# sanderslab/magellanmapper

Measured on AMD Instinct MI355X. Metric: Mvoxels/s, 2048x2048x1024 uint16 stack, 5-sigma LoG blob detection, higher is better.
Workload: dtype f16x2 MFMA (f32 accumulate) + 16-bit fixed-point intermediates; f64 re-score of every candidate

## Files before the change

### magellanmapper_amd/csrc/mmx_api.hip

```cpp

#include <atomic>
#include <cstdio>
#include <cstdlib>
#include <cstring>

#include "mmx_common.h"

int mmx_launch_generic_pass(int pass, const mmx_volume* vol, const mmx_block* d_blocks, int n_blocks,
                            int max_vox, int64_t slot_elems, const float* w0, const float* w2, int radius,
                            const float* in1, const float* in2, float* out1, float* out2, hipStream_t s);
int mmx_launch_peaks(const float* d_log, int n_sigma, int64_t sigma_stride, const mmx_block* d_blocks,
                     int n_blocks, int max_vox, int64_t slot_elems, float thr, float eps,
                     mmx_cand* d_cands, uint32_t cap, uint32_t* d_count, hipStream_t stream);
int mmx_launch_peaks_sparse(const float* d_log, const unsigned long long* d_mask, int n_sigma,
                            int64_t sigma_stride, const mmx_block* d_blocks, int n_blocks, int max_vox,
                            int64_t slot_elems, float thr, float eps, mmx_cand* d_cands, uint32_t cap,
                            uint32_t* d_count, int quads, hipStream_t stream);

#include <mutex>
#include <vector>

namespace {
thread_local char g_hip_err[256] = "";

// ... 211 lines not shown
    int kind; hipStream_t s;
    pass_scope(int k, hipStream_t st) : kind(k), s(st) { if (k >= 0) mmx_time_begin(k, st); }
    ~pass_scope() { if (kind >= 0) mmx_time_end(kind, s); }
};

int fused_passes(const mmx_log_call& c, const mmx_route& r, const mmx_batch_geom& g, const pass_weights& w)
{
    const mmx_volume* vol = c.vol;
    const int radius = c.radius, n_blocks = c.n_blocks;
    const int64_t slot_elems = c.slot_elems;
    hipStream_t s = c.stream;
    float* t0 = c.d_work;
    float* t1 = c.d_work + (int64_t)n_blocks * slot_elems;
    mmx_taps_f32 tzz = taps(w.z0, w.z2, radius), txx = taps(w.y0, w.y2, radius), tyy = taps(w.x0, w.x2, radius);
    const bool tiled = r.family == MMX_ROUTE_TILED;
    const mmx_zx6_plan& plan = g.plan;
    int rc;
    if (r.makes_copy) {
        mmx_timed_scope ts(MMX_K_ZXPACK, s);
        rc = mmx_launch_zx6_pack(vol, c.d_blocks, c.h_blocks, n_blocks, plan, c.d_work, s);
        if (rc != MMX_OK) return launched(rc, "mmx_launch_zx6_pack", "voxel copy of the tiled path");
    }
    { mmx_timed_scope ts(MMX_K_ZX, s);
      if (tiled)
          rc = mmx_launch_zx6(vol, c.d_blocks, c.h_blocks, n_blocks, plan, txx, radius, c.d_work,
                              r.q16 ? (float)(1.0 / r.bp) : 0.f, r.q16 ? (float)(1.0 / r.bq) : 0.f, s);
      else
          rc = mmx_launch_zx2(vol, c.d_blocks, n_blocks, g.max_ny, g.max_px, slot_elems, tzz, txx, radius, t0, t1, s); }
    if (rc != MMX_OK) return launched(rc, tiled ? "mmx_launch_zx6" : "mmx_launch_zx2", "fused passes");
    { mmx_timed_scope ts(MMX_K_Y2, s);
      unsigned long long* d_mask = r.layout ? (unsigned long long*)c.d_nms_mask : nullptr;
      const float cp = r.q16 ? (float)(r.bp / 65535.0) : 0.f, cq = r.q16 ? (float)(r.bq / 32767.0) : 0.f;
      if (r.y_kernel == MMX_Y_YM)
          rc = mmx_launch_ym(c.d_blocks, n_blocks, plan, slot_elems, tyy, radius, c.d_work, cp, cq, c.d_log, d_mask,
                             c.nms_lo, c.nms_eps, s);
      else if (r.y_kernel == MMX_Y_Y6)
          rc = mmx_launch_y6(c.d_blocks, n_blocks, plan, slot_elems, tyy, radius, c.d_work,
                             reinterpret_cast<const float*>(reinterpret_cast<const char*>(c.d_work) + plan.q_off), cp, cq,
                             c.d_log, d_mask, c.nms_lo, c.nms_eps, s);
      else
          rc = mmx_launch_y2(c.d_blocks, n_blocks, g.max_ycols, slot_elems, tyy, radius, t0, t1, c.d_log, d_mask, c.nms_lo,
                             c.nms_eps, s); }
    return launched(rc, r.y_kernel == MMX_Y_YM ? "mmx_launch_ym" : (r.y_kernel == MMX_Y_Y6 ? "mmx_launch_y6" : "mmx_launch_y2"),
                    "fused passes");
}

int wide_passes(const mmx_log_call& c, const mmx_route& r, const pass_weights& w)
{
    const int radius = c.radius, n_blocks = c.n_blocks;
    const int64_t slot_elems = c.slot_elems;
    hipStream_t s = c.stream;
    float* t0 = c.d_work;
    float* t1 = t0 + (int64_t)n_blocks * slot_elems;
    float* t2 = t1 + (int64_t)n_blocks * slot_elems;
    float* t3 = t2 + (int64_t)n_blocks * slot_elems;
    unsigned long long* d_mask = r.layout ? (unsigned long long*)c.d_nms_mask : nullptr;
    int rc;
    { mmx_timed_scope ts(MMX_K_WIDE, s);
      rc = mmx_launch_wide_pass(0, c.vol, c.d_blocks, c.h_blocks, n_blocks, slot_elems, w.z0, w.z2, radius, nullptr, nullptr,
                                t2, t3, nullptr, 0.f, 0.f, s); }
    if (rc == MMX_OK) {
        mmx_timed_scope ts(MMX_K_WIDE, s);
        rc = mmx_launch_wide_pass(1, c.vol, c.d_blocks, c.h_blocks, n_blocks, slot_elems, w.y0, w.y2, radius, t2, t3, t0, t1,
                                  nullptr, 0.f, 0.f, s);
    }
    if (rc == MMX_OK) {
        mmx_timed_scope ts(MMX_K_WIDE, s);
// ... 196 lines not shown
```

### magellanmapper_amd/csrc/mmx_common.h

```cpp
#pragma once

#include <hip/hip_runtime.h>
#include <stdint.h>

#include "../../include/mmx.h"

#define MMX_WG 256
#define MMX_MAX_GRID_X 2147483647

struct mmx_taps_f32 {
    float w0[MMX_MAX_RADIUS_FAST + 1];
    float w2[MMX_MAX_RADIUS_FAST + 1];
};

__host__ __device__ __forceinline__ int mmx_reflect(int i, int n)
{
    if (n == 1) return 0;
    const int period = 2 * n;
    i %= period;
    if (i < 0) i += period;
    return i < n ? i : period - 1 - i;
}

int mmx_launch_zpass(const mmx_volume* vol, const mmx_block* d_blocks, int n_blocks, int max_cols,
                     int64_t slot_elems, const mmx_taps_f32& taps, int radius,
                     float* d_gz, float* d_gzz, hipStream_t stream);
int mmx_launch_ypass(const mmx_block* d_blocks, int n_blocks, int max_cols, int64_t slot_elems,
                     const mmx_taps_f32& taps, int radius, const float* d_gz, const float* d_gzz,
                     float* d_a, float* d_bc, hipStream_t stream);
int mmx_launch_xpass(const mmx_block* d_blocks, int n_blocks, int max_rows, int max_nx,
                     int64_t slot_elems, const mmx_taps_f32& taps, int radius,
                     const float* d_a, const float* d_bc, float* d_log, hipStream_t stream);

int mmx_launch_zx2(const mmx_volume* vol, const mmx_block* d_blocks, int n_blocks, int max_ny, int max_px,
                   int64_t slot_elems, const mmx_taps_f32& tz, const mmx_taps_f32& tx, int radius,
                   float* d_p, float* d_q, hipStream_t s);
struct mmx_zx6_plan {
    int64_t tile_stride;
    int64_t pack_stride;
    int64_t q_off, tab_off, pack_off;
    int64_t tab_bytes;
    int max_tiles;
    int max_rowtiles;
};
int mmx_zx6_plan_make(const mmx_block* h_blocks, int n_blocks, int64_t slot_elems, int voxel_dtype, mmx_zx6_plan* plan);
int mmx_launch_zx6_pack(const mmx_volume* vol, const mmx_block* d_blocks, const mmx_block* h_blocks, int n_blocks,
                        const mmx_zx6_plan& plan, void* d_work, hipStream_t stream);
int mmx_launch_zx6(const mmx_volume* vol, const mmx_block* d_blocks, const mmx_block* h_blocks, int n_blocks,
                   const mmx_zx6_plan& plan, const mmx_taps_f32& tx, int radius, void* d_work, float qp, float qq,
                   hipStream_t stream);
int mmx_launch_y6(const mmx_block* d_blocks, int n_blocks, const mmx_zx6_plan& plan, int64_t slot_elems,
                  const mmx_taps_f32& taps, int radius, const float* d_p, const float* d_q, float cp, float cq,
                  float* d_log, unsigned long long* d_mask, float nms_lo, float nms_eps, hipStream_t stream);
int mmx_launch_ym(const mmx_block* d_blocks, int n_blocks, const mmx_zx6_plan& plan, int64_t slot_elems,
                  const mmx_taps_f32& taps, int radius, const float* d_p, float cp, float cq,
                  float* d_log, unsigned long long* d_mask, float nms_lo, float nms_eps, hipStream_t stream);
int mmx_launch_y2(const mmx_block* d_blocks, int n_blocks, int max_cols, int64_t slot_elems,
                  const mmx_taps_f32& taps, int radius, const float* d_p, const float* d_q,
                  float* d_log, unsigned long long* d_mask, float nms_lo, float nms_eps, hipStream_t stream);

int mmx_launch_wide_pass(int pass, const mmx_volume* vol, const mmx_block* d_blocks, const mmx_block* h_blocks, int n_blocks,
                         int64_t slot_elems, const float* w0, const float* w2, int radius,
                         const float* in1, const float* in2, float* out1, float* out2,
                         unsigned long long* d_mask, float nms_lo, float nms_eps, hipStream_t s);

struct mmx_batch_geom {
    int status;
    bool bad_block;
    int min_nz, min_ny, min_nx, max_ny, max_nx, max_px;
    int max_zcols, max_ycols, max_rows, max_vox;
    int64_t max_lane_in;
    bool rows_fit, quads_fit;
    mmx_zx6_plan plan;
    int plan_status;
};
void mmx_batch_geom_make(const mmx_volume* vol, const mmx_block* h_blocks, int n_blocks, int64_t slot_elems, mmx_batch_geom* g);

#include "mmx_route.h"

struct mmx_log_call {
    const mmx_volume* vol; const mmx_block* d_blocks; const mmx_block* h_blocks; int n_blocks; int64_t slot_elems;
    const double* h_w0; const double* h_w2; int radius; double norm;
    float* d_log; float* d_work; uint64_t* d_nms_mask; float nms_lo, nms_eps; int* h_mask_written;
    int zx_mode; int* h_zx_path; hipStream_t stream;
};
int mmx_log_scale_check(const mmx_log_call& c);
int mmx_log_scale_run(const mmx_log_call& c, const mmx_batch_geom& g, const mmx_route& r);
int mmx_zx_pack_geom(const mmx_volume* vol, const mmx_block* d_blocks, const mmx_block* h_blocks, int n_blocks,
// ... 16 lines not shown
```

### magellanmapper_amd/csrc/mmx_fused4.hip

```cpp

#include <algorithm>
#include <type_traits>

#include "mmx_common.h"

typedef _Float16 h2_4 __attribute__((ext_vector_type(2)));
typedef _Float16 h8_4 __attribute__((ext_vector_type(8)));
typedef float f2_4 __attribute__((ext_vector_type(2)));
typedef float f4_4 __attribute__((ext_vector_type(4)));
typedef unsigned u4_4 __attribute__((ext_vector_type(4)));
typedef unsigned u2_4 __attribute__((ext_vector_type(2)));

#define MMX_ZX4_MAXCLS 8
#ifndef ZX4_ST_AUX
#define ZX4_ST_AUX 0
#endif
#ifndef ZX4_LD_AUX
#define ZX4_LD_AUX 0
#endif

struct mmx_zx4_cfg {
    float w0[MMX_MAX_RADIUS_FAST + 1];
    float w2[MMX_MAX_RADIUS_FAST + 1];
    float xscale;
// ... 28 lines not shown
template <int NKX, int LA> struct cls4 {
    static constexpr int R8 = NKX == 1 ? 8 : (LA == 1 ? 16 : 24);
    static __host__ __device__ constexpr int xstart(int c)
    {
        const int lo = 16 * c - R8;
        const int al = lo & ~31;
        return (al + 32 * NKX >= 16 * c + 16 + R8) ? al : lo;
    }
    static constexpr bool SPLIT = LA == 2;
    static constexpr int NKZ = 2;
    static constexpr int NT = 4;
};

__device__ __forceinline__ unsigned pack_h2(float a, float b)
{
    const f2_4 v = {a, b};
    return __builtin_bit_cast(unsigned, __builtin_convertvector(v, h2_4));
}

__device__ __forceinline__ float folded_tap(const float* w, int R, int p, int o, int n)
{
    float s = 0.f;
    int d = p - o; d = d < 0 ? -d : d;
    if (d <= R) s += w[d];
    d = (-1 - p) - o; d = d < 0 ? -d : d;
    if (d <= R) s += w[d];
    d = (2 * n - 1 - p) - o; d = d < 0 ? -d : d;
    if (d <= R) s += w[d];
    return s;
}

template <int NKX, int LA>
__global__ void __launch_bounds__(256)
zx4_setup(mmx_zx4_cfg cfg, u4_4* __restrict__ xtab, u4_4* __restrict__ ztab)
{
    using cg = cls4<NKX, LA>;
    const int R = cfg.radius;
    const int lane = threadIdx.x & 63;
    const int kq = lane >> 4, col = lane & 15;
    const int e = blockIdx.x * 4 + (threadIdx.x >> 6);
    const int nx_entries = cfg.ncw * cfg.maxcol * NKX * 2;
    const int nz_entries = cfg.ncz * cfg.maxu * cg::NKZ * 2;
    float wt[8];
    u4_4* dst;
    if (e < nx_entries) {
        const int kern = e & 1;
        const int m = (e >> 1) % NKX;
        const int c = ((e >> 1) / NKX) % cfg.maxcol;
        const int cl = ((e >> 1) / NKX) / cfg.maxcol;
        const int W = cfg.wcls[cl];
        const float* w = kern ? cfg.w2 : cfg.w0;
        const int xo = 16 * c + col;
        const int cwin = cfg.ntw == 2 ? (c & ~1) : c;
        const int xc = (cfg.staged == 2 ? 16 * cwin - cg::R8 : cg::xstart(c)) + 32 * m + 8 * kq;
        int xl = xc < 0 ? 0 : xc;
        xl = xl > W - 8 ? W - 8 : xl;
        if (cfg.staged) xl = xc;
#pragma unroll
        for (int j = 0; j < 8; ++j) {
            const int p = xl + j;
            const bool ok = p >= xc && p < xc + 8 && p >= 0 && p < W && xo < W;
            wt[j] = ok ? folded_tap(w, R, p, xo, W) * cfg.xscale * (cfg.qp > 0.f ? (kern ? cfg.qq : cfg.qp) : 1.f) : 0.f;
        }
        dst = xtab + (size_t)e * 2 * 64;
    } else if (e < nx_entries + nz_entries) {
        const int ez = e - nx_entries;
        const int kern = ez & 1;
        const int ks = (ez >> 1) % cg::NKZ;
// ... 650 lines not shown
{
    using cg = cls4<NKX, LA>;
    mmx_zx4_cfg cfg{};
    for (int k = 0; k <= MMX_MAX_RADIUS_FAST; ++k) { cfg.w0[k] = tx.w0[k]; cfg.w2[k] = tx.w2[k]; }
    cfg.radius = radius;
    cfg.xscale = vol->dtype == MMX_U16 ? (float)(65536.0 / 65535.0) :
                 (vol->dtype == MMX_U8 ? (float)(65536.0 / (255.0 * 256.0)) : 1.f);
    cfg.staged = 2;
    cfg.qp = qp; cfg.qq = qq;
    const bool pair = NKX == 2 && LA == 1 && qp > 0.f && vol->dtype != MMX_F32;
    cfg.ntw = pair ? 2 : 1;
    zx_classes cl;
    if (!collect_classes(h_blocks, n_blocks, &cl)) return MMX_ERR_UNSUPPORTED;
    cfg.ncw = cl.ncw; cfg.ncz = cl.ncz; cfg.maxcol = cl.maxcol; cfg.maxu = cl.maxu;
    for (int j = 0; j < MMX_ZX4_MAXCLS; ++j) {
        cfg.wcls[j] = j < cl.ncw ? cl.wcls[j] : -1;
        cfg.zcls[j] = j < cl.ncz ? cl.zcls[j] : -1;
    }
    int max_waves = 0;
    for (int i = 0; i < n_blocks; ++i) {
        const mmx_block& b = h_blocks[i];
        if (!mmx_zx6_launch_accepts(vol, b.nz, b.nx, radius)) return MMX_ERR_UNSUPPORTED;
        const int ntx = (b.nx + 15) / 16;
        max_waves = std::max(max_waves, b.ny * (pair ? (ntx + 1) / 2 : ntx));
    }
    const int nx_entries = cfg.ncw * cfg.maxcol * NKX * 2;
    const int nz_entries = cfg.ncz * cfg.maxu * cg::NKZ * 2;
    const size_t xbytes = (size_t)nx_entries * 2 * 64 * sizeof(u4_4);
    const size_t zbytes = (size_t)nz_entries * 2 * 64 * sizeof(u4_4);
    if ((int64_t)(xbytes + zbytes) > plan.tab_bytes) return MMX_ERR_UNSUPPORTED;
    char* w = reinterpret_cast<char*>(d_work);
    u4_4* xtab = reinterpret_cast<u4_4*>(w + plan.tab_off);
    u4_4* ztab = reinterpret_cast<u4_4*>(w + plan.tab_off + xbytes);
    hipLaunchKernelGGL((zx4_setup<NKX, LA>), dim3((nx_entries + nz_entries + 3) / 4), dim3(256), 0, s, cfg, xtab, ztab);
    dim3 grid((((max_waves + 3) / 4) + 7) & ~7, n_blocks);
    if (vol->dtype == MMX_F32) {
        if (qp > 0.f)
            hipLaunchKernelGGL((zx4_kernel<NKX, LA, float, true>), grid, dim3(256), 0, s,
                               reinterpret_cast<const float*>(w + plan.pack_off), plan.pack_stride / 2, (int64_t)0, d_blocks,
                               plan.tile_stride, reinterpret_cast<float*>(w), reinterpret_cast<float*>(w + plan.q_off),
                               xtab, ztab, cfg);
        else
            hipLaunchKernelGGL((zx4_kernel<NKX, LA, float, false>), grid, dim3(256), 0, s,
                               reinterpret_cast<const float*>(w + plan.pack_off), plan.pack_stride / 2, (int64_t)0, d_blocks,
                               plan.tile_stride, reinterpret_cast<float*>(w), reinterpret_cast<float*>(w + plan.q_off),
                               xtab, ztab, cfg);
    } else if (pair) {
        if constexpr (NKX == 2 && LA == 1)
            hipLaunchKernelGGL((zx4_kernel<NKX, LA, uint16_t, true, 2>), grid, dim3(256), 0, s,
                               reinterpret_cast<const uint16_t*>(w + plan.pack_off), plan.pack_stride, (int64_t)0, d_blocks,
                               plan.tile_stride, reinterpret_cast<float*>(w), reinterpret_cast<float*>(w + plan.q_off),
                               xtab, ztab, cfg);
    } else if (qp > 0.f)
        hipLaunchKernelGGL((zx4_kernel<NKX, LA, uint16_t, true>), grid, dim3(256), 0, s,
                           reinterpret_cast<const uint16_t*>(w + plan.pack_off), plan.pack_stride, (int64_t)0, d_blocks,
                           plan.tile_stride, reinterpret_cast<float*>(w), reinterpret_cast<float*>(w + plan.q_off),
                           xtab, ztab, cfg);
    else
        hipLaunchKernelGGL((zx4_kernel<NKX, LA, uint16_t, false>), grid, dim3(256), 0, s,
                           reinterpret_cast<const uint16_t*>(w + plan.pack_off), plan.pack_stride, (int64_t)0, d_blocks,
                           plan.tile_stride, reinterpret_cast<float*>(w), reinterpret_cast<float*>(w + plan.q_off),
                           xtab, ztab, cfg);
    return hipGetLastError() == hipSuccess ? MMX_OK : MMX_ERR_HIP;
}

}

// ... 65 lines not shown
```

### magellanmapper_amd/csrc/mmx_ymfma.hip

```cpp

#include <type_traits>

#include <cstdlib>

#include "mmx_common.h"

typedef _Float16 h2_y __attribute__((ext_vector_type(2)));
typedef _Float16 h8_y __attribute__((ext_vector_type(8)));
typedef float f2_y __attribute__((ext_vector_type(2)));
typedef float f4_y __attribute__((ext_vector_type(4)));
typedef unsigned u4_y __attribute__((ext_vector_type(4)));

struct ym_cfg {
    float w2[MMX_MAX_RADIUS_FAST + 1];
    float w0[MMX_MAX_RADIUS_FAST + 1];
    float unscale;
    float start;
    float lo, eps;
    int radius;
    int reverse;
};

namespace {

using rsrc_y = __amdgpu_buffer_rsrc_t;
__device__ __forceinline__ rsrc_y make_rsrc_y(const void* p)
{
    return __builtin_amdgcn_make_buffer_rsrc(const_cast<void*>(p), 0, 0x7fffffff, 0x00020000);
}
__device__ __forceinline__ unsigned pack_h2y(float a, float b)
{
    const f2_y v = {a, b};
    return __builtin_bit_cast(unsigned, __builtin_convertvector(v, h2_y));
}
__device__ __forceinline__ f4_y mfma_y(const u4_y& a, const u4_y& b, const f4_y& c)
{
    return __builtin_amdgcn_mfma_f32_16x16x32_f16(__builtin_bit_cast(h8_y, a), __builtin_bit_cast(h8_y, b), c, 0, 0, 0);
}

#ifndef YM5_OCC
#define YM5_OCC 2
#endif
#ifndef YM6_WAVES
#define YM6_WAVES 4
#define YM6_JH 4
#define YM6_NF 4
#endif
template <int NB, bool MASK>
__global__ void __launch_bounds__(NB <= 4 ? 256 : YM6_WAVES * 64, NB <= 4 ? 3 : (YM6_WAVES == 4 ? YM5_OCC : 1))
ym_kernel(const mmx_block* __restrict__ blocks, int64_t slot_elems, int64_t tile_stride,
          const unsigned* __restrict__ gt, float* __restrict__ out, ym_cfg cfg,
          unsigned long long* __restrict__ mask)
{
    constexpr int RB = 8 * (NB - 2);
    constexpr int NF = NB <= 4 ? 4 : YM6_NF;
    __shared__ u4_y frag[NB * NF * 64];
    constexpr int WAVES = NB <= 4 ? 4 : YM6_WAVES;
    constexpr int JH = NB <= 4 ? 4 : YM6_JH;
    __shared__ float tr[WAVES * 2 * 1024];

    const mmx_block bd = blocks[cfg.reverse ? gridDim.y - 1 - blockIdx.y : blockIdx.y];
    const int ntx = (bd.nx + 15) >> 4, ntz = (bd.nz + 15) >> 4;
    if ((int)blockIdx.x * (WAVES / 4) >= ntx * ntz) return;
    for (int e = threadIdx.x; e < NB * NF * 64; e += WAVES * 64) {
        const int ln = e & 63, f = e >> 6;
        const int piece = (f % NF) % (NF / 2), kern = (f % NF) / (NF / 2), t = f / NF;
        const int m = ln & 15, kq = ln >> 4;
        const int delta = RB - 16 * t;
        unsigned pk[4];
#pragma unroll
        for (int i = 0; i < 8; i += 2) {
            float v[2];
#pragma unroll
            for (int u = 0; u < 2; ++u) {
                int d = 8 * kq + i + u - m + delta;
                d = d < 0 ? -d : d;
                const float ws = d <= cfg.radius ? (kern ? cfg.w0[d] : cfg.w2[d]) : 0.f;
                const float h = (float)(_Float16)ws;
                v[u] = piece == 0 ? h : (piece == 1 ? (ws - h) * 256.f : h * 256.f);
            }
            pk[i >> 1] = pack_h2y(v[0], v[1]);
        }
        frag[e] = (u4_y){pk[0], pk[1], pk[2], pk[3]};
    }
    __syncthreads();

    const int wv = __builtin_amdgcn_readfirstlane((int)(threadIdx.x >> 6));
    const int tile = (int)blockIdx.x * (WAVES / 4) + (wv >> 2);
    if (tile >= ntx * ntz) return;
    const int c = tile / ntz, U = tile - c * ntz;
    const int zq = wv & 3;
    if (16 * U + 4 * zq >= bd.nz) return;
    const int lane = threadIdx.x & 63;
    const int n = bd.ny;
    const float nms_lo = cfg.lo, nms_eps = cfg.eps, us = cfg.unscale;
    const int kq = lane >> 4, n16 = lane & 15;
    const unsigned trow_b = (unsigned)(ntx * ntz) * 1024u;
    const rsrc_y rs = make_rsrc_y(gt + (int64_t)bd.slot * tile_stride + (int64_t)tile * 256);
    const unsigned voff = (unsigned)(zq * 256 + n16 * 16);
    const unsigned voff_s = voff + (unsigned)(8 * kq) * trow_b;
    const int xi = lane & 15;
    const int z = 16 * U + 4 * zq + (lane >> 4), x = 16 * c + xi;
    const bool real = z < bd.nz && x < bd.nx;
    float* w1 = out + (int64_t)bd.slot * slot_elems;
    const rsrc_y rsw = make_rsrc_y(w1);
    const unsigned ooff = (unsigned)((real ? z : 0) * bd.ny * bd.px + (real ? x : 0)) * 4u;
    const unsigned row_b = (unsigned)bd.px * 4u;
    const int nent = ((bd.nz + 3) >> 2) * ntx;
    ulonglong2* mrow = MASK ? reinterpret_cast<ulonglong2*>(mask) + ((int64_t)bd.slot * slot_elems >> 5) +
                              (4 * U + zq) * ntx + c
                            : nullptr;
    unsigned long long ab_prev = 0;
    const bool has_l = xi > 0, has_r = xi < 15 && x + 1 < bd.nx;
    float prev1 = -INFINITY, prev2 = -INFINITY, nbx_prev = -INFINITY;
    int ydone = 0;
    float* trw = tr + wv * 2048;

    auto row = [&](float acc, int y) __attribute__((always_inline)) {
        const unsigned long long ab = MASK ? __ballot(real & (acc > nms_lo)) : ~0ull;
#ifndef YM_NOSTORE
        if (ab && real) __builtin_amdgcn_raw_buffer_store_b32(__float_as_uint(acc * us), rsw, ooff, (unsigned)y * row_b, 0);
#endif
        if constexpr (MASK) {
            float nbx = -INFINITY;
            if (ab) {
                const float l = __uint_as_float((unsigned)__builtin_amdgcn_update_dpp(
                    (int)__float_as_uint(acc), (int)__float_as_uint(acc), 0x111 , 0xf, 0xf, false));
                const float rr = __uint_as_float((unsigned)__builtin_amdgcn_update_dpp(
                    (int)__float_as_uint(acc), (int)__float_as_uint(acc), 0x101 , 0xf, 0xf, false));
                nbx = fmaxf(has_l ? l : -INFINITY, has_r ? rr : -INFINITY);
            }
            if (ydone > 0) {
                unsigned long long m = 0;
                if (ab_prev) {
                    const bool cand = real & (prev1 > nms_lo) &
                                      !(fmaxf(fmaxf(prev2, acc), nbx_prev) > prev1 + nms_eps);
                    m = __ballot(cand);
                }
                if (lane == 0) *mrow = make_ulonglong2(m, ab_prev);
                mrow += nent;
            }
            prev2 = prev1; prev1 = acc; nbx_prev = nbx;
            ab_prev = ab;
            ++ydone;
        }
    };
    auto rows_of = [&](int T, int s, bool any) __attribute__((always_inline)) {
        if (T < 0 || 16 * T >= n) return;
        const int cnt = n - 16 * T < 16 ? n - 16 * T : 16;
        if (MASK && !any) {
            if (ydone > 0) {
                unsigned long long m = 0;
                if (ab_prev) {
                    const bool cand = real & (prev1 > nms_lo) & !(fmaxf(prev2, nbx_prev) > prev1 + nms_eps);
                    m = __ballot(cand);
                }
                if (lane == 0) *mrow = make_ulonglong2(m, ab_prev);
                mrow += nent;
            }
            if (lane < cnt - 1) mrow[(int64_t)lane * nent] = make_ulonglong2(0ull, 0ull);
            mrow += (int64_t)(cnt - 1) * nent;
            prev1 = prev2 = nbx_prev = -INFINITY;
            ab_prev = 0;
            ydone += cnt;
            return;
        }
        const float* src = trw + s * 1024 + lane;
        if (!MASK || cnt < 16) {
#pragma unroll 1
            for (int r = 0; r < cnt; ++r) row(src[r * 64], 16 * T + r);
            return;
        }
        float v[16];
#pragma unroll
        for (int r = 0; r < 16; ++r) v[r] = src[r * 64];
        unsigned long long ab[16];
        unsigned long long some = 0;
#pragma unroll
        for (int r = 0; r < 16; ++r) { ab[r] = __ballot(real & (v[r] > nms_lo)); some |= ab[r]; }
        unsigned e0 = 0, e1 = 0, e2 = 0, e3 = 0;
        auto put = [&](int ln, unsigned long long m, unsigned long long a) __attribute__((always_inline)) {
            const bool me = lane == ln;
            e0 = me ? (unsigned)m : e0;
            e1 = me ? (unsigned)(m >> 32) : e1;
            e2 = me ? (unsigned)a : e2;
            e3 = me ? (unsigned)(a >> 32) : e3;
        };
        if (ab_prev) {
            const bool cand = real & (prev1 > nms_lo) & !(fmaxf(fmaxf(prev2, v[0]), nbx_prev) > prev1 + nms_eps);
            put(0, __ballot(cand), ab_prev);
        }
        float nbx15 = -INFINITY;
        if (some) {
#pragma unroll
            for (int r = 0; r < 16; ++r) {
                if (ab[r]) {
#ifndef YM_NOSTORE
                    if (real) __builtin_amdgcn_raw_buffer_store_b32(__float_as_uint(v[r] * us), rsw, ooff, (unsigned)(16 * T + r) * row_b, 0);
#endif
                    const float l = __uint_as_float((unsigned)__builtin_amdgcn_update_dpp(
                        (int)__float_as_uint(v[r]), (int)__float_as_uint(v[r]), 0x111 , 0xf, 0xf, false));
                    const float rr = __uint_as_float((unsigned)__builtin_amdgcn_update_dpp(
                        (int)__float_as_uint(v[r]), (int)__float_as_uint(v[r]), 0x101 , 0xf, 0xf, false));
                    const float nbx = fmaxf(has_l ? l : -INFINITY, has_r ? rr : -INFINITY);
                    if (r < 15) {
                        const float below = r > 0 ? v[r > 0 ? r - 1 : 0] : prev1;
                        const bool cand = real & (v[r] > nms_lo) & !(fmaxf(fmaxf(below, v[r < 15 ? r + 1 : 15]), nbx) > v[r] + nms_eps);
                        put(r + 1, __ballot(cand), ab[r]);
                    } else {
                        nbx15 = nbx;
                    }
                }
            }
        }
        if (lane < 16 && (lane > 0 || ydone > 0)) {
            ulonglong2* dst = mrow + (int64_t)(ydone > 0 ? lane : lane - 1) * nent;
            *dst = make_ulonglong2((unsigned long long)e0 | ((unsigned long long)e1 << 32),
                                   (unsigned long long)e2 | ((unsigned long long)e3 << 32));
        }
        mrow += (int64_t)(ydone > 0 ? 16 : 15) * nent;
        prev2 = v[14]; prev1 = v[15]; nbx_prev = nbx15;
        ab_prev = ab[15];
        ydone += 16;
    };

#ifndef YM_PFD
#define YM_PFD 1
#endif
    constexpr int PFD = YM_PFD;
    u4_y rawA[8], rawB[PFD == 2 ? 8 : 1];
    auto load_block = [&](int b, u4_y (&raw)[8]) __attribute__((always_inline)) {
        const int r0 = -RB + 32 * b;
        if (r0 >= 0 && r0 + 32 <= n) {
#pragma unroll
            for (int i = 0; i < 8; ++i)
                raw[i] = __builtin_bit_cast(u4_y, __builtin_amdgcn_raw_buffer_load_b128(rs, voff_s, (unsigned)(r0 + i) * trow_b, 0));
        } else {
#pragma unroll
            for (int i = 0; i < 8; ++i) {
                int v = r0 + 8 * kq + i;
                v = v < 0 ? -1 - v : v;
                v = v >= n ? 2 * n - 1 - v : v;
                v = v < 0 ? 0 : (v > n - 1 ? n - 1 : v);
                raw[i] = __builtin_bit_cast(u4_y, __builtin_amdgcn_raw_buffer_load_b128(rs, voff + (unsigned)v * trow_b, 0, 0));
            }
        }
    };
    const int nT = (n + 15) >> 4;
    const int nKB = (nT + NB - 3) / 2 + 1;
    const f4_y start = {cfg.start, cfg.start, cfg.start, cfg.start};
    f4_y acc[NB][4];
#pragma unroll
    for (int t = 0; t < NB; ++t)
#pragma unroll
        for (int j = 0; j < 4; ++j) acc[t][j] = start;
    bool any0 = false, any1 = false;

    const _Float16 k256 = (_Float16)256.f;
    auto iter = [&](int b, u4_y (&raw)[8]) __attribute__((always_inline)) {
#ifndef YM_ROWS_LATE
#define YM_ROWS_LATE 1
#endif
        if (!YM_ROWS_LATE || b == nKB) {
#pragma unroll 1
            for (int h = 0; h < 2; ++h) rows_of(2 * (b - 1) - NB + 2 + h, h, h ? any1 : any0);
        }
        if (b == nKB) return false;
        if constexpr (JH < 4) { any0 = !MASK; any1 = !MASK; }
#pragma unroll
        for (int j0 = 0; j0 < 4; j0 += JH) {
            __builtin_amdgcn_sched_barrier(0);
            u4_y pc[JH][4];
#pragma unroll
            for (int j = 0; j < JH; ++j)
#pragma unroll
                for (int p = 0; p < 4; ++p) {
                    const unsigned d0 = raw[2 * p][j0 + j], d1 = raw[2 * p + 1][j0 + j];
                    pc[j][0][p] = __builtin_amdgcn_perm(d1, d0, 0x0c050c01u);
                    pc[j][1][p] = __builtin_amdgcn_perm(d1, d0, 0x0c040c00u);
                    pc[j][2][p] = __builtin_amdgcn_perm(d1, d0, 0x0c070c03u) ^ 0x00800080u;
                    pc[j][3][p] = __builtin_amdgcn_perm(d1, d0, 0x0c060c02u);
                }
            __builtin_amdgcn_sched_barrier(0);
            if (j0 + JH == 4 && b + PFD < nKB) load_block(b + PFD, raw);
            __builtin_amdgcn_sched_barrier(0);
            if (YM_ROWS_LATE && JH == 4) {
#pragma unroll 1
                for (int h = 0; h < 2; ++h) rows_of(2 * (b - 1) - NB + 2 + h, h, h ? any1 : any0);
                __builtin_amdgcn_sched_barrier(0);
            }
            auto tile_mfmas = [&](int t, bool fresh) __attribute__((always_inline)) {
                f4_y* a = &acc[t][j0];
                const u4_y* fr = frag + (t * NF) * 64 + lane;
                const u4_y ah = fr[0], al = fr[64], bh = fr[(NF / 2) * 64], bl = fr[(NF / 2 + 1) * 64];
                const u4_y a256 = NF == 6 ? fr[128] : __builtin_bit_cast(u4_y, __builtin_bit_cast(h8_y, ah) * k256);
                const u4_y b256 = NF == 6 ? fr[320] : __builtin_bit_cast(u4_y, __builtin_bit_cast(h8_y, bh) * k256);
#pragma unroll
                for (int j = 0; j < JH; ++j) a[j] = mfma_y(a256, pc[j][0], fresh ? start : a[j]);
#pragma unroll
                for (int j = 0; j < JH; ++j) a[j] = mfma_y(ah, pc[j][1], a[j]);
#pragma unroll
                for (int j = 0; j < JH; ++j) a[j] = mfma_y(al, pc[j][0], a[j]);
#pragma unroll
                for (int j = 0; j < JH; ++j) a[j] = mfma_y(b256, pc[j][2], a[j]);
#pragma unroll
                for (int j = 0; j < JH; ++j) a[j] = mfma_y(bh, pc[j][3], a[j]);
#pragma unroll
                for (int j = 0; j < JH; ++j) a[j] = mfma_y(bl, pc[j][2], a[j]);
            };
#pragma unroll
            for (int t = 0; t < 2; ++t) tile_mfmas(t, t >= NB - 2);
#pragma unroll
            for (int t = 0; t < 2; ++t) {
                const f4_y* a = &acc[t][j0];
                float mx = -INFINITY;
#pragma unroll
                for (int j = 0; j < JH; ++j)
#pragma unroll
                    for (int r = 0; r < 4; ++r) mx = fmaxf(mx, a[j][r]);
                const bool any = MASK ? __ballot(mx > nms_lo) != 0ull : true;
                if constexpr (JH == 4) {
                    if (t == 0) any0 = any; else any1 = any;
                    if (any) {
                        f4_y* dst = reinterpret_cast<f4_y*>(trw + t * 1024) + (4 * kq) * 16 + n16;
#pragma unroll
                        for (int r = 0; r < 4; ++r) dst[r * 16] = (f4_y){a[0][r], a[1][r], a[2][r], a[3][r]};
                    }
                } else {
                    if (t == 0) any0 |= any; else any1 |= any;
                    f2_y* dst = reinterpret_cast<f2_y*>(trw + t * 1024) + (4 * kq) * 32 + 2 * n16 + (j0 >> 1);
#pragma unroll
                    for (int r = 0; r < 4; ++r) dst[r * 32] = (f2_y){a[0][r], a[1][r]};
                }
            }
            __builtin_amdgcn_sched_barrier(0);
#pragma unroll
            for (int t = 2; t < NB; ++t) {
                tile_mfmas(t, t >= NB - 2);
                if constexpr (NB > 4) __builtin_amdgcn_sched_barrier(0);
            }
        }
#pragma unroll
        for (int t = 0; t + 2 < NB; ++t)
#pragma unroll
            for (int j = 0; j < 4; ++j) acc[t][j] = acc[t + 2][j];
        __builtin_amdgcn_wave_barrier();
        return true;
    };
    load_block(0, rawA);
    if constexpr (PFD == 2) {
        if (nKB > 1) load_block(1, reinterpret_cast<u4_y (&)[8]>(rawB));
#pragma unroll 1
        for (int b = 0;; b += 2) {
            if (!iter(b, rawA)) break;
            if (!iter(b + 1, reinterpret_cast<u4_y (&)[8]>(rawB))) break;
        }
    } else {
#pragma unroll 1
        for (int b = 0; iter(b, rawA); ++b) {}
    }
    if constexpr (MASK) {
        unsigned long long m = 0;
        if (ab_prev) {
            const bool cand = real & (prev1 > nms_lo) & !(fmaxf(prev2, nbx_prev) > prev1 + nms_eps);
            m = __ballot(cand);
        }
        if (lane == 0) *mrow = make_ulonglong2(m, ab_prev);
    }
}

template <int NB>
int launch_ym(const mmx_block* d_blocks, int n_blocks, const mmx_zx6_plan& plan, int64_t slot_elems,
              const ym_cfg& cfg, const float* d_p, float* d_log, unsigned long long* d_mask, hipStream_t s)
{
    constexpr int TPW = NB <= 4 ? 1 : YM6_WAVES / 4;
    dim3 grid((plan.max_tiles + TPW - 1) / TPW, n_blocks);
    if (d_mask)
        hipLaunchKernelGGL((ym_kernel<NB, true>), grid, dim3(256 * TPW), 0, s, d_blocks, slot_elems, plan.tile_stride,
                           reinterpret_cast<const unsigned*>(d_p), d_log, cfg, d_mask);
    else
        hipLaunchKernelGGL((ym_kernel<NB, false>), grid, dim3(256 * TPW), 0, s, d_blocks, slot_elems, plan.tile_stride,
                           reinterpret_cast<const unsigned*>(d_p), d_log, cfg, d_mask);
    return hipGetLastError() == hipSuccess ? MMX_OK : MMX_ERR_HIP;
}

}

int mmx_launch_ym(const mmx_block* d_blocks, int n_blocks, const mmx_zx6_plan& plan, int64_t slot_elems,
                  const mmx_taps_f32& taps, int radius, const float* d_p, float cp, float cq,
                  float* d_log, unsigned long long* d_mask, float nms_lo, float nms_eps, hipStream_t stream)
{
    if (!mmx_ym_accepts(taps.w0, taps.w2, radius, cp, cq)) return MMX_ERR_UNSUPPORTED;
    ym_cfg cfg;
    float mx = 0.f;
    for (int k = 0; k <= radius; ++k) {
        cfg.w2[k] = taps.w2[k] * cp;
        cfg.w0[k] = taps.w0[k] * cq;
        mx = fmaxf(mx, fmaxf(fabsf(cfg.w2[k]), fabsf(cfg.w0[k])));
    }
    int e;
    frexpf(mx, &e);
    const float up = ldexpf(1.f, -e - 1);
    double q128 = 0.0;
    for (int k = 0; k <= MMX_MAX_RADIUS_FAST; ++k) {
        cfg.w2[k] = k <= radius ? cfg.w2[k] * up : 0.f;
        cfg.w0[k] = k <= radius ? cfg.w0[k] * up : 0.f;
        const float h = (float)(_Float16)cfg.w0[k];
        const float l = (float)(_Float16)((cfg.w0[k] - h) * 256.f);
        q128 += (k ? 2.0 : 1.0) * ((double)h * 256.0 + (double)l);
    }
    cfg.start = (float)(-128.0 * 0x1p-24 * q128);
    cfg.unscale = ldexpf(1.f, e + 1 + 24);
    cfg.lo = nms_lo / cfg.unscale;
    cfg.eps = nms_eps / cfg.unscale;
    cfg.radius = radius;
    cfg.reverse = 1;
    if (radius <= 8) return launch_ym<3>(d_blocks, n_blocks, plan, slot_elems, cfg, d_p, d_log, d_mask, stream);
    if (radius <= 16) return launch_ym<4>(d_blocks, n_blocks, plan, slot_elems, cfg, d_p, d_log, d_mask, stream);
    return launch_ym<5>(d_blocks, n_blocks, plan, slot_elems, cfg, d_p, d_log, d_mask, stream);
}
```

Measured before the change: 44460.

## Make the y-pass MFMA kernel persistent with an atomic work-ticket queue

Replaces the per-tile 2D grid of the YM y-pass kernel with a persistent grid sized to resident occupancy. Each wave pulls wave-sized units (a 16-column by 4-z slab) from a global atomic ticket, and the ticket is reset in the zx4 setup kernel. While finishing the current unit, a wave prefetches the first row block of its next unit, overlapping the tail of one unit with the loads of the next. This aims to remove idle waves and tail imbalance from ragged tiles and to hide load latency between units. The cost is per-wave atomics, a linear block-search cursor, more register state, and reuse of the q_off workspace region as the ticket.

```diff
diff --git a/magellanmapper_amd/csrc/mmx_api.hip b/magellanmapper_amd/csrc/mmx_api.hip
--- a/magellanmapper_amd/csrc/mmx_api.hip
+++ b/magellanmapper_amd/csrc/mmx_api.hip
@@ -267,7 +267,7 @@
       unsigned long long* d_mask = r.layout ? (unsigned long long*)c.d_nms_mask : nullptr;
       const float cp = r.q16 ? (float)(r.bp / 65535.0) : 0.f, cq = r.q16 ? (float)(r.bq / 32767.0) : 0.f;
       if (r.y_kernel == MMX_Y_YM)
-          rc = mmx_launch_ym(c.d_blocks, n_blocks, plan, slot_elems, tyy, radius, c.d_work, cp, cq, c.d_log, d_mask,
+          rc = mmx_launch_ym(c.d_blocks, c.h_blocks, n_blocks, plan, slot_elems, tyy, radius, c.d_work, cp, cq, c.d_log, d_mask,
                              c.nms_lo, c.nms_eps, s);
       else if (r.y_kernel == MMX_Y_Y6)
           rc = mmx_launch_y6(c.d_blocks, n_blocks, plan, slot_elems, tyy, radius, c.d_work,
diff --git a/magellanmapper_amd/csrc/mmx_common.h b/magellanmapper_amd/csrc/mmx_common.h
--- a/magellanmapper_amd/csrc/mmx_common.h
+++ b/magellanmapper_amd/csrc/mmx_common.h
@@ -52,8 +52,8 @@
 int mmx_launch_y6(const mmx_block* d_blocks, int n_blocks, const mmx_zx6_plan& plan, int64_t slot_elems,
                   const mmx_taps_f32& taps, int radius, const float* d_p, const float* d_q, float cp, float cq,
                   float* d_log, unsigned long long* d_mask, float nms_lo, float nms_eps, hipStream_t stream);
-int mmx_launch_ym(const mmx_block* d_blocks, int n_blocks, const mmx_zx6_plan& plan, int64_t slot_elems,
-                  const mmx_taps_f32& taps, int radius, const float* d_p, float cp, float cq,
+int mmx_launch_ym(const mmx_block* d_blocks, const mmx_block* h_blocks, int n_blocks, const mmx_zx6_plan& plan,
+                  int64_t slot_elems, const mmx_taps_f32& taps, int radius, float* d_work, float cp, float cq,
                   float* d_log, unsigned long long* d_mask, float nms_lo, float nms_eps, hipStream_t stream);
 int mmx_launch_y2(const mmx_block* d_blocks, int n_blocks, int max_cols, int64_t slot_elems,
                   const mmx_taps_f32& taps, int radius, const float* d_p, const float* d_q,
diff --git a/magellanmapper_amd/csrc/mmx_fused4.hip b/magellanmapper_amd/csrc/mmx_fused4.hip
--- a/magellanmapper_amd/csrc/mmx_fused4.hip
+++ b/magellanmapper_amd/csrc/mmx_fused4.hip
@@ -84,8 +84,9 @@
 
 template <int NKX, int LA>
 __global__ void __launch_bounds__(256)
-zx4_setup(mmx_zx4_cfg cfg, u4_4* __restrict__ xtab, u4_4* __restrict__ ztab)
-{
+zx4_setup(mmx_zx4_cfg cfg, u4_4* __restrict__ xtab, u4_4* __restrict__ ztab, unsigned* __restrict__ ym_ticket)
+{
+    if (ym_ticket && blockIdx.x == 0 && threadIdx.x == 0) *ym_ticket = 0u;
     using cg = cls4<NKX, LA>;
     const int R = cfg.radius;
     const int lane = threadIdx.x & 63;
@@ -802,7 +803,8 @@
     char* w = reinterpret_cast<char*>(d_work);
     u4_4* xtab = reinterpret_cast<u4_4*>(w + plan.tab_off);
     u4_4* ztab = reinterpret_cast<u4_4*>(w + plan.tab_off + xbytes);
-    hipLaunchKernelGGL((zx4_setup<NKX, LA>), dim3((nx_entries + nz_entries + 3) / 4), dim3(256), 0, s, cfg, xtab, ztab);
+    hipLaunchKernelGGL((zx4_setup<NKX, LA>), dim3((nx_entries + nz_entries + 3) / 4), dim3(256), 0, s, cfg, xtab, ztab,
+                       qp > 0.f ? reinterpret_cast<unsigned*>(w + plan.q_off) : nullptr);
     dim3 grid((((max_waves + 3) / 4) + 7) & ~7, n_blocks);
     if (vol->dtype == MMX_F32) {
         if (qp > 0.f)
diff --git a/magellanmapper_amd/csrc/mmx_ym_units.h b/magellanmapper_amd/csrc/mmx_ym_units.h
--- /dev/null
+++ b/magellanmapper_amd/csrc/mmx_ym_units.h
@@ -0,0 +1,48 @@
+#pragma once
+
+#include <hip/hip_runtime.h>
+#include <stdint.h>
+
+#include "../../include/mmx.h"
+
+__host__ __device__ __forceinline__ int mmx_ym_block_units(int nz, int nx)
+{
+    return ((nx + 15) >> 4) * ((nz + 3) >> 2);
+}
+
+__host__ __device__ __forceinline__ int mmx_ym_block_at(int pos, int n_blocks, int reverse)
+{
+    return reverse ? n_blocks - 1 - pos : pos;
+}
+
+__host__ __device__ inline int64_t mmx_ym_unit_count(const mmx_block* blocks, int n_blocks)
+{
+    int64_t total = 0;
+    for (int i = 0; i < n_blocks; ++i) total += mmx_ym_block_units(blocks[i].nz, blocks[i].nx);
+    return total;
+}
+
+struct mmx_ym_cursor { int pos, base; };
+struct mmx_ym_unit { int block, tile, zq, c; };
+
+__host__ __device__ __forceinline__ bool mmx_ym_unit_at(const mmx_block* blocks, int n_blocks, int reverse, int u,
+                                                        mmx_ym_cursor* cur, mmx_ym_unit* out)
+{
+    for (; cur->pos < n_blocks; ++cur->pos) {
+        const int bi = mmx_ym_block_at(cur->pos, n_blocks, reverse);
+        const int nz = blocks[bi].nz;
+        const int cnt = mmx_ym_block_units(nz, blocks[bi].nx);
+        const int r = u - cur->base;
+        if (r < cnt) {
+            const int nzq = (nz + 3) >> 2, ntz = (nz + 15) >> 4;
+            const int c = r / nzq, q = r - c * nzq;
+            out->block = bi;
+            out->c = c;
+            out->tile = c * ntz + (q >> 2);
+            out->zq = q & 3;
+            return true;
+        }
+        cur->base += cnt;
+    }
+    return false;
+}
diff --git a/magellanmapper_amd/csrc/mmx_ymfma.hip b/magellanmapper_amd/csrc/mmx_ymfma.hip
--- a/magellanmapper_amd/csrc/mmx_ymfma.hip
+++ b/magellanmapper_amd/csrc/mmx_ymfma.hip
@@ -1,9 +1,11 @@
 
+#include <algorithm>
+#include <atomic>
+#include <cstdlib>
 #include <type_traits>
 
-#include <cstdlib>
-
 #include "mmx_common.h"
+#include "mmx_ym_units.h"
 
 typedef _Float16 h2_y __attribute__((ext_vector_type(2)));
 typedef _Float16 h8_y __attribute__((ext_vector_type(8)));
@@ -48,8 +50,8 @@
 #endif
 template <int NB, bool MASK>
 __global__ void __launch_bounds__(NB <= 4 ? 256 : YM6_WAVES * 64, NB <= 4 ? 3 : (YM6_WAVES == 4 ? YM5_OCC : 1))
-ym_kernel(const mmx_block* __restrict__ blocks, int64_t slot_elems, int64_t tile_stride,
-          const unsigned* __restrict__ gt, float* __restrict__ out, ym_cfg cfg,
+ym_kernel(const mmx_block* __restrict__ blocks, int n_blocks, int total, unsigned* __restrict__ ticket,
+          int64_t slot_elems, int64_t tile_stride, const unsigned* __restrict__ gt, float* __restrict__ out, ym_cfg cfg,
           unsigned long long* __restrict__ mask)
 {
     constexpr int RB = 8 * (NB - 2);
@@ -59,9 +61,55 @@
     constexpr int JH = NB <= 4 ? 4 : YM6_JH;
     __shared__ float tr[WAVES * 2 * 1024];
 
-    const mmx_block bd = blocks[cfg.reverse ? gridDim.y - 1 - blockIdx.y : blockIdx.y];
-    const int ntx = (bd.nx + 15) >> 4, ntz = (bd.nz + 15) >> 4;
-    if ((int)blockIdx.x * (WAVES / 4) >= ntx * ntz) return;
+    const int wv = __builtin_amdgcn_readfirstlane((int)(threadIdx.x >> 6));
+    const int lane = threadIdx.x & 63;
+    const int kq = lane >> 4, n16 = lane & 15;
+    auto ask = [&]() __attribute__((always_inline)) {
+        unsigned t = 0;
+        if (lane == 0) t = __hip_atomic_fetch_add(ticket, 1u, __ATOMIC_RELAXED, __HIP_MEMORY_SCOPE_AGENT);
+        return t;
+    };
+    auto take = [&](unsigned t) __attribute__((always_inline)) { return __builtin_amdgcn_readfirstlane((int)t); };
+    mmx_ym_cursor cur = {0, 0};
+    rsrc_y rs = make_rsrc_y(gt);
+    unsigned zq_b = 0, trow_b = 0;
+    int n_ld = 1;
+    auto loads_to = [&](int u) __attribute__((always_inline)) {
+        mmx_ym_unit un;
+        if ((unsigned)u >= (unsigned)total || !mmx_ym_unit_at(blocks, n_blocks, cfg.reverse, u, &cur, &un)) return false;
+        const mmx_block& bd = blocks[un.block];
+        trow_b = (unsigned)(((bd.nx + 15) >> 4) * ((bd.nz + 15) >> 4)) * 1024u;
+        rs = make_rsrc_y(gt + (int64_t)bd.slot * tile_stride + (int64_t)un.tile * 256);
+        zq_b = (unsigned)un.zq * 256u;
+        n_ld = bd.ny;
+        return true;
+    };
+    u4_y rawA[8];
+    auto load_block = [&](int b, u4_y (&raw)[8]) __attribute__((always_inline)) {
+        int l = lane;
+        asm volatile("" : "+v"(l));
+        const int k8 = 8 * (l >> 4);
+        const unsigned voff = zq_b + (unsigned)(l & 15) * 16u;
+        const int r0 = -RB + 32 * b;
+        if (r0 >= 0 && r0 + 32 <= n_ld) {
+            const unsigned voff_s = voff + (unsigned)k8 * trow_b;
+#pragma unroll
+            for (int i = 0; i < 8; ++i)
+                raw[i] = __builtin_bit_cast(u4_y, __builtin_amdgcn_raw_buffer_load_b128(rs, voff_s, (unsigned)(r0 + i) * trow_b, 0));
+        } else {
+#pragma unroll
+            for (int i = 0; i < 8; ++i) {
+                int v = r0 + k8 + i;
+                v = v < 0 ? -1 - v : v;
+                v = v >= n_ld ? 2 * n_ld - 1 - v : v;
+                v = v < 0 ? 0 : (v > n_ld - 1 ? n_ld - 1 : v);
+                raw[i] = __builtin_bit_cast(u4_y, __builtin_amdgcn_raw_buffer_load_b128(rs, voff + (unsigned)v * trow_b, 0, 0));
+            }
+        }
+    };
+    int unit = take(ask());
+    const bool have = loads_to(unit);
+    if (have) load_block(0, rawA);
     for (int e = threadIdx.x; e < NB * NF * 64; e += WAVES * 64) {
         const int ln = e & 63, f = e >> 6;
         const int piece = (f % NF) % (NF / 2), kern = (f % NF) / (NF / 2), t = f / NF;
@@ -85,36 +133,52 @@
     }
     __syncthreads();
 
-    const int wv = __builtin_amdgcn_readfirstlane((int)(threadIdx.x >> 6));
-    const int tile = (int)blockIdx.x * (WAVES / 4) + (wv >> 2);
-    if (tile >= ntx * ntz) return;
-    const int c = tile / ntz, U = tile - c * ntz;
-    const int zq = wv & 3;
-    if (16 * U + 4 * zq >= bd.nz) return;
-    const int lane = threadIdx.x & 63;
-    const int n = bd.ny;
+    if (!have) return;
     const float nms_lo = cfg.lo, nms_eps = cfg.eps, us = cfg.unscale;
-    const int kq = lane >> 4, n16 = lane & 15;
-    const unsigned trow_b = (unsigned)(ntx * ntz) * 1024u;
-    const rsrc_y rs = make_rsrc_y(gt + (int64_t)bd.slot * tile_stride + (int64_t)tile * 256);
-    const unsigned voff = (unsigned)(zq * 256 + n16 * 16);
-    const unsigned voff_s = voff + (unsigned)(8 * kq) * trow_b;
+    const f4_y start = {cfg.start, cfg.start, cfg.start, cfg.start};
     const int xi = lane & 15;
-    const int z = 16 * U + 4 * zq + (lane >> 4), x = 16 * c + xi;
-    const bool real = z < bd.nz && x < bd.nx;
-    float* w1 = out + (int64_t)bd.slot * slot_elems;
-    const rsrc_y rsw = make_rsrc_y(w1);
-    const unsigned ooff = (unsigned)((real ? z : 0) * bd.ny * bd.px + (real ? x : 0)) * 4u;
-    const unsigned row_b = (unsigned)bd.px * 4u;
-    const int nent = ((bd.nz + 3) >> 2) * ntx;
-    ulonglong2* mrow = MASK ? reinterpret_cast<ulonglong2*>(mask) + ((int64_t)bd.slot * slot_elems >> 5) +
-                              (4 * U + zq) * ntx + c
-                            : nullptr;
+    const bool has_l = xi > 0;
+    int n = 1, nKB = 1;
+    bool real = false, has_r = false;
+    rsrc_y rsw = make_rsrc_y(out);
+    unsigned ooff = 0, row_b = 0;
+    int nent = 0;
+    ulonglong2* mrow = nullptr;
     unsigned long long ab_prev = 0;
-    const bool has_l = xi > 0, has_r = xi < 15 && x + 1 < bd.nx;
     float prev1 = -INFINITY, prev2 = -INFINITY, nbx_prev = -INFINITY;
     int ydone = 0;
+    bool any0 = false, any1 = false;
+    f4_y acc[NB][4];
     float* trw = tr + wv * 2048;
+    auto rows_to = [&](int u) __attribute__((always_inline)) {
+        mmx_ym_unit un;
+        if (!mmx_ym_unit_at(blocks, n_blocks, cfg.reverse, u, &cur, &un)) return false;
+        const mmx_block& bd = blocks[un.block];
+        const int ntx = (bd.nx + 15) >> 4, ntz = (bd.nz + 15) >> 4;
+        const int U = un.tile - un.c * ntz;
+        const int z = 16 * U + 4 * un.zq + (lane >> 4), x = 16 * un.c + xi;
+        n = bd.ny;
+        const int nT = (n + 15) >> 4;
+        nKB = (nT + NB - 3) / 2 + 1;
+        real = z < bd.nz && x < bd.nx;
+        has_r = xi < 15 && x + 1 < bd.nx;
+        rsw = make_rsrc_y(out + (int64_t)bd.slot * slot_elems);
+        ooff = (unsigned)((real ? z : 0) * bd.ny * bd.px + (real ? x : 0)) * 4u;
+        row_b = (unsigned)bd.px * 4u;
+        nent = ((bd.nz + 3) >> 2) * ntx;
+        mrow = MASK ? reinterpret_cast<ulonglong2*>(mask) + ((int64_t)bd.slot * slot_elems >> 5) +
+                      (4 * U + un.zq) * ntx + un.c
+                    : nullptr;
+        ab_prev = 0;
+        prev1 = prev2 = nbx_prev = -INFINITY;
+        ydone = 0;
+        any0 = any1 = false;
+#pragma unroll
+        for (int t = 0; t < NB; ++t)
+#pragma unroll
+            for (int j = 0; j < 4; ++j) acc[t][j] = start;
+        return true;
+    };
 
     auto row = [&](float acc, int y) __attribute__((always_inline)) {
         const unsigned long long ab = MASK ? __ballot(real & (acc > nms_lo)) : ~0ull;
@@ -179,8 +243,10 @@
 #pragma unroll
         for (int r = 0; r < 16; ++r) { ab[r] = __ballot(real & (v[r] > nms_lo)); some |= ab[r]; }
         unsigned e0 = 0, e1 = 0, e2 = 0, e3 = 0;
+        int lq = lane;
+        asm volatile("" : "+v"(lq));
         auto put = [&](int ln, unsigned long long m, unsigned long long a) __attribute__((always_inline)) {
-            const bool me = lane == ln;
+            const bool me = lq == ln;
             e0 = me ? (unsigned)m : e0;
             e1 = me ? (unsigned)(m >> 32) : e1;
             e2 = me ? (unsigned)a : e2;
@@ -224,40 +290,8 @@
         ydone += 16;
     };
 
-#ifndef YM_PFD
-#define YM_PFD 1
-#endif
-    constexpr int PFD = YM_PFD;
-    u4_y rawA[8], rawB[PFD == 2 ? 8 : 1];
-    auto load_block = [&](int b, u4_y (&raw)[8]) __attribute__((always_inline)) {
-        const int r0 = -RB + 32 * b;
-        if (r0 >= 0 && r0 + 32 <= n) {
-#pragma unroll
-            for (int i = 0; i < 8; ++i)
-                raw[i] = __builtin_bit_cast(u4_y, __builtin_amdgcn_raw_buffer_load_b128(rs, voff_s, (unsigned)(r0 + i) * trow_b, 0));
-        } else {
-#pragma unroll
-            for (int i = 0; i < 8; ++i) {
-                int v = r0 + 8 * kq + i;
-                v = v < 0 ? -1 - v : v;
-                v = v >= n ? 2 * n - 1 - v : v;
-                v = v < 0 ? 0 : (v > n - 1 ? n - 1 : v);
-                raw[i] = __builtin_bit_cast(u4_y, __builtin_amdgcn_raw_buffer_load_b128(rs, voff + (unsigned)v * trow_b, 0, 0));
-            }
-        }
-    };
-    const int nT = (n + 15) >> 4;
-    const int nKB = (nT + NB - 3) / 2 + 1;
-    const f4_y start = {cfg.start, cfg.start, cfg.start, cfg.start};
-    f4_y acc[NB][4];
-#pragma unroll
-    for (int t = 0; t < NB; ++t)
-#pragma unroll
-        for (int j = 0; j < 4; ++j) acc[t][j] = start;
-    bool any0 = false, any1 = false;
-
     const _Float16 k256 = (_Float16)256.f;
-    auto iter = [&](int b, u4_y (&raw)[8]) __attribute__((always_inline)) {
+    auto iter = [&](int b, u4_y (&raw)[8], int& next, unsigned& asked) __attribute__((always_inline)) {
 #ifndef YM_ROWS_LATE
 #define YM_ROWS_LATE 1
 #endif
@@ -266,6 +300,11 @@
             for (int h = 0; h < 2; ++h) rows_of(2 * (b - 1) - NB + 2 + h, h, h ? any1 : any0);
         }
         if (b == nKB) return false;
+        if (b + 1 == nKB) {
+            if (nKB == 1) asked = ask();
+            next = take(asked);
+            if (!loads_to(next)) next = total;
+        }
         if constexpr (JH < 4) { any0 = !MASK; any1 = !MASK; }
 #pragma unroll
         for (int j0 = 0; j0 < 4; j0 += JH) {
@@ -282,7 +321,11 @@
                     pc[j][3][p] = __builtin_amdgcn_perm(d1, d0, 0x0c060c02u);
                 }
             __builtin_amdgcn_sched_barrier(0);
-            if (j0 + JH == 4 && b + PFD < nKB) load_block(b + PFD, raw);
+            if (j0 + JH == 4) {
+                const bool last = b + 1 >= nKB;
+                if (!last || (unsigned)next < (unsigned)total) load_block(last ? 0 : b + 1, raw);
+                if (b + 2 == nKB) asked = ask();
+            }
             __builtin_amdgcn_sched_barrier(0);
             if (YM_ROWS_LATE && JH == 4) {
 #pragma unroll 1
@@ -292,6 +335,9 @@
             auto tile_mfmas = [&](int t, bool fresh) __attribute__((always_inline)) {
                 f4_y* a = &acc[t][j0];
                 const u4_y* fr = frag + (t * NF) * 64 + lane;
+                float st = cfg.start;
+                asm volatile("" : "+s"(st));
+                const f4_y start = {st, st, st, st};
                 const u4_y ah = fr[0], al = fr[64], bh = fr[(NF / 2) * 64], bl = fr[(NF / 2 + 1) * 64];
                 const u4_y a256 = NF == 6 ? fr[128] : __builtin_bit_cast(u4_y, __builtin_bit_cast(h8_y, ah) * k256);
                 const u4_y b256 = NF == 6 ? fr[320] : __builtin_bit_cast(u4_y, __builtin_bit_cast(h8_y, bh) * k256);
@@ -347,47 +393,79 @@
         __builtin_amdgcn_wave_barrier();
         return true;
     };
-    load_block(0, rawA);
-    if constexpr (PFD == 2) {
-        if (nKB > 1) load_block(1, reinterpret_cast<u4_y (&)[8]>(rawB));
+    for (;;) {
+        if (!rows_to(unit)) break;
+        int next = total;
+        unsigned asked = 0;
 #pragma unroll 1
-        for (int b = 0;; b += 2) {
-            if (!iter(b, rawA)) break;
-            if (!iter(b + 1, reinterpret_cast<u4_y (&)[8]>(rawB))) break;
-        }
-    } else {
-#pragma unroll 1
-        for (int b = 0; iter(b, rawA); ++b) {}
+        for (int b = 0; iter(b, rawA, next, asked); ++b) {}
+        if constexpr (MASK) {
+            unsigned long long m = 0;
+            if (ab_prev) {
+                const bool cand = real & (prev1 > nms_lo) & !(fmaxf(prev2, nbx_prev) > prev1 + nms_eps);
+                m = __ballot(cand);
+            }
+            if (lane == 0) *mrow = make_ulonglong2(m, ab_prev);
+        }
+        if ((unsigned)next >= (unsigned)total) break;
+        unit = next;
     }
-    if constexpr (MASK) {
-        unsigned long long m = 0;
-        if (ab_prev) {
-            const bool cand = real & (prev1 > nms_lo) & !(fmaxf(prev2, nbx_prev) > prev1 + nms_eps);
-            m = __ballot(cand);
-        }
-        if (lane == 0) *mrow = make_ulonglong2(m, ab_prev);
+}
+
+constexpr int kMaxDev = 64;
+template <int NB, bool MASK>
+int ym_resident()
+{
+    static std::atomic<int> known[kMaxDev];
+    int dev = 0;
+    if (hipGetDevice(&dev) != hipSuccess) return -1;
+    const bool slot = dev >= 0 && dev < kMaxDev;
+    int v = slot ? known[dev].load(std::memory_order_relaxed) : 0;
+    if (v > 0) return v;
+    constexpr int threads = NB <= 4 ? 256 : YM6_WAVES * 64;
+    int per_cu = 0, cus = 0;
+    if (hipOccupancyMaxActiveBlocksPerMultiprocessor(&per_cu, ym_kernel<NB, MASK>, threads, 0) != hipSuccess ||
+        hipDeviceGetAttribute(&cus, hipDeviceAttributeMultiprocessorCount, dev) != hipSuccess || per_cu < 1 || cus < 1)
+        return -1;
+    v = per_cu * cus;
+    if (slot) known[dev].store(v, std::memory_order_relaxed);
+    return v;
+}
+
+template <int NB, bool MASK>
+int launch_ym_as(const mmx_block* d_blocks, int n_blocks, int64_t total, unsigned* ticket, const mmx_zx6_plan& plan,
+                 int64_t slot_elems, const ym_cfg& cfg, const float* d_p, float* d_log, unsigned long long* d_mask,
+                 hipStream_t s)
+{
+    constexpr int WAVES = NB <= 4 ? 4 : YM6_WAVES;
+    const int resident = ym_resident<NB, MASK>();
+    if (resident < 1) return MMX_ERR_HIP;
+    int64_t wgs = std::min<int64_t>(resident, std::max<int64_t>(total / WAVES, 1));
+    if (const char* env = getenv("MMX_YM_WORKGROUPS")) {
+        const long cap = atol(env);
+        if (cap > 0 && cap < wgs) wgs = cap;
     }
+    if (total + wgs * WAVES >= (int64_t(1) << 31)) return MMX_ERR_UNSUPPORTED;
+    hipLaunchKernelGGL((ym_kernel<NB, MASK>), dim3((unsigned)wgs), dim3(WAVES * 64), 0, s, d_blocks, n_blocks, (int)total,
+                       ticket, slot_elems, plan.tile_stride, reinterpret_cast<const unsigned*>(d_p), d_log, cfg, d_mask);
+    return hipGetLastError() == hipSuccess ? MMX_OK : MMX_ERR_HIP;
 }
 
 template <int NB>
-int launch_ym(const mmx_block* d_blocks, int n_blocks, const mmx_zx6_plan& plan, int64_t slot_elems,
-              const ym_cfg& cfg, const float* d_p, float* d_log, unsigned long long* d_mask, hipStream_t s)
-{
-    constexpr int TPW = NB <= 4 ? 1 : YM6_WAVES / 4;
-    dim3 grid((plan.max_tiles + TPW - 1) / TPW, n_blocks);
-    if (d_mask)
-        hipLaunchKernelGGL((ym_kernel<NB, true>), grid, dim3(256 * TPW), 0, s, d_blocks, slot_elems, plan.tile_stride,
-                           reinterpret_cast<const unsigned*>(d_p), d_log, cfg, d_mask);
-    else
-        hipLaunchKernelGGL((ym_kernel<NB, false>), grid, dim3(256 * TPW), 0, s, d_blocks, slot_elems, plan.tile_stride,
-                           reinterpret_cast<const unsigned*>(d_p), d_log, cfg, d_mask);
-    return hipGetLastError() == hipSuccess ? MMX_OK : MMX_ERR_HIP;
-}
-
-}
-
-int mmx_launch_ym(const mmx_block* d_blocks, int n_blocks, const mmx_zx6_plan& plan, int64_t slot_elems,
-                  const mmx_taps_f32& taps, int radius, const float* d_p, float cp, float cq,
+int launch_ym(const mmx_block* d_blocks, const mmx_block* h_blocks, int n_blocks, const mmx_zx6_plan& plan,
+              int64_t slot_elems, const ym_cfg& cfg, float* d_work, float* d_log, unsigned long long* d_mask, hipStream_t s)
+{
+    const int64_t total = mmx_ym_unit_count(h_blocks, n_blocks);
+    if (total < 1) return MMX_OK;
+    unsigned* ticket = reinterpret_cast<unsigned*>(reinterpret_cast<char*>(d_work) + plan.q_off);
+    return d_mask ? launch_ym_as<NB, true>(d_blocks, n_blocks, total, ticket, plan, slot_elems, cfg, d_work, d_log, d_mask, s)
+                  : launch_ym_as<NB, false>(d_blocks, n_blocks, total, ticket, plan, slot_elems, cfg, d_work, d_log, d_mask, s);
+}
+
+}
+
+int mmx_launch_ym(const mmx_block* d_blocks, const mmx_block* h_blocks, int n_blocks, const mmx_zx6_plan& plan,
+                  int64_t slot_elems, const mmx_taps_f32& taps, int radius, float* d_work, float cp, float cq,
                   float* d_log, unsigned long long* d_mask, float nms_lo, float nms_eps, hipStream_t stream)
 {
     if (!mmx_ym_accepts(taps.w0, taps.w2, radius, cp, cq)) return MMX_ERR_UNSUPPORTED;
@@ -415,7 +493,7 @@
     cfg.eps = nms_eps / cfg.unscale;
     cfg.radius = radius;
     cfg.reverse = 1;
-    if (radius <= 8) return launch_ym<3>(d_blocks, n_blocks, plan, slot_elems, cfg, d_p, d_log, d_mask, stream);
-    if (radius <= 16) return launch_ym<4>(d_blocks, n_blocks, plan, slot_elems, cfg, d_p, d_log, d_mask, stream);
-    return launch_ym<5>(d_blocks, n_blocks, plan, slot_elems, cfg, d_p, d_log, d_mask, stream);
-}
+    if (radius <= 8) return launch_ym<3>(d_blocks, h_blocks, n_blocks, plan, slot_elems, cfg, d_work, d_log, d_mask, stream);
+    if (radius <= 16) return launch_ym<4>(d_blocks, h_blocks, n_blocks, plan, slot_elems, cfg, d_work, d_log, d_mask, stream);
+    return launch_ym<5>(d_blocks, h_blocks, n_blocks, plan, slot_elems, cfg, d_work, d_log, d_mask, stream);
+}
```

Result: no change. 44150 (-0.7%).
